# MeteoSwiss/topo-descriptors

Measured on AMD Instinct MI355X. Metric: Mpixels/s (and % HBM roofline) per descriptor, 1/2/4/8 MI355X, higher is better.
Workload: dtype f32

## Files before the change

### topo_descriptors_amd/csrc/disc_ring_wide_impl.hpp

```cpp
#pragma once

namespace topo {

namespace {

constexpr int NCW = 6;

template <int SIZE>
struct WGeo {
    static constexpr DiscTable<SIZE> T = make_disc_table<SIZE>();
    static_assert(T.centre == 0 && T.off_min == -T.off_max, "odd disc sizes only");
    static constexpr int M = T.off_max;
    static constexpr int DL = (M + NCW - 1) / NCW;
    static constexpr int NVL = 64 - 2 * DL;
    static constexpr int TILE_W = NCW * NVL;
    static constexpr int X0 = NCW * DL;
    static constexpr int W = 64 * NCW;
    static constexpr int NR = T.num_runs;
    static_assert(NVL >= 16, "disc too wide for one wavefront");
    struct Sched {
        int first_step[SIZE];
        int order[SIZE];
        int centre_run;
    };
    static constexpr Sched make() {
        Sched t{};
        for (int r = 0; r < SIZE; ++r) t.first_step[r] = -1;
        for (int r = 0; r < SIZE; ++r) t.order[r] = 0;
        t.centre_run = -1;
        for (int D = 0; D <= DL; ++D)
            for (int s = 0; s < NCW; ++s)
                for (int q = 0; q < NCW; ++q) {
                    const int dr = NCW * D + s - q, dl = -NCW * D + s - q;
                    if (dr >= 0 && dr <= M) {
                        const int r = T.run_of[dr - T.off_min];
                        if (D > t.first_step[r]) t.first_step[r] = D;
                    }
                    if (dl < 0 && dl >= -M) {
                        const int r = T.run_of[dl - T.off_min];
                        if (D > t.first_step[r]) t.first_step[r] = D;
                    }
                }
        int n = 0;
        for (int D = DL; D >= 0; --D)
            for (int d = M; d >= 0; --d) {
                const int r = T.run_of[d - T.off_min];
                bool seen = false;
                for (int i = 0; i < n; ++i) seen = seen || t.order[i] == r;
                if (!seen && t.first_step[r] == D) t.order[n++] = r;
            }
        for (int r = 0; r < NR; ++r)
            if (T.run_lo[r] == 0 && T.run_hi[r] == 0) t.centre_run = r;
        return t;
    }
    static constexpr Sched S = make();
    static_assert(S.centre_run >= 0, "the disc's outermost column is the pixel's own row");
};

template <int SIZE>
struct WideCfg {
    using G = WGeo<SIZE>;
    static constexpr int SW = 3;
    static constexpr int CW = 8;
    static constexpr int NW = SW + CW;
    static constexpr int RPW = 2;
    static constexpr int B = CW * RPW;
    static constexpr int TH = 64;
    static constexpr int PPT = TH / B;
    static constexpr int R = SIZE + 2 * B;
    static constexpr int GR = 6;
    static constexpr int HALO = SIZE - 1;
    static constexpr int PAD = 1 + (B - (1 + HALO + B) % B) % B;
    static constexpr int PRO = PAD + HALO + B;
    static constexpr int NB_PRO = PRO / B;
    static constexpr size_t LDS = (size_t)(R + GR) * G::W * sizeof(uint32_t) + 2 * SW * sizeof(int) + 16;
    static_assert(SW * 128 == G::W, "two staged columns per staging lane");
    static_assert(TH % B == 0 && PRO % B == 0, "whole batches");
    static_assert(LDS <= 160 * 1024, "ring does not fit LDS");
    static_assert(NB_PRO <= 15, "batch history: two fields of a flag word");
};

constexpr bool tpi_wide_ring_fits(int size) {
    return size >= 5 && size % 2 == 1 && (size_t)(size + 32 + 6) * 384 * 4 + 64 <= 160 * 1024 && 64 - 2 * ((size / 2 + 5) / 6) >= 16;
}

template <int SIZE, int GR>
struct WBase {
    using G = WGeo<SIZE>;
    static constexpr int NR = G::NR;
    struct Tab {
        int nb;
        int kb[2 * SIZE];
        int first[2 * SIZE];
        int top_b[SIZE], bot_b[SIZE];
        int top_k[SIZE], bot_k[SIZE];
    };
    static constexpr Tab make() {
        Tab t{};
        bool need[2 * SIZE + 2] = {};
        for (int i = 0; i < NR; ++i) {
            const int r = G::S.order[i];
            t.top_k[i] = G::T.run_hi[r] + 1 + G::M;
            t.bot_k[i] = G::T.run_lo[r] + G::M;
            need[t.top_k[i]] = need[t.bot_k[i]] = true;
        }
        t.nb = 0;
        for (int k = 0; k <= 2 * G::M + 1; ++k)
            if (need[k] && (t.nb == 0 || k > t.kb[t.nb - 1] + GR)) t.kb[t.nb++] = k;
        for (int b = 0; b < t.nb; ++b) t.first[b] = NR;
        auto base_of = [&](int k) {
            int b = 0;
            while (b + 1 < t.nb && t.kb[b + 1] <= k) ++b;
            return b;
        };
        for (int i = 0; i < NR; ++i) {
            t.top_b[i] = base_of(t.top_k[i]);
            t.bot_b[i] = base_of(t.bot_k[i]);
            if (i < t.first[t.top_b[i]]) t.first[t.top_b[i]] = i;
            if (i < t.first[t.bot_b[i]]) t.first[t.bot_b[i]] = i;
        }
        return t;
    }
    static constexpr Tab T = make();
    static constexpr bool check() {
        for (int i = 0; i < NR; ++i)
            if (T.top_k[i] - T.kb[T.top_b[i]] > GR || T.top_k[i] < T.kb[T.top_b[i]] || T.bot_k[i] - T.kb[T.bot_b[i]] > GR ||
                T.bot_k[i] < T.kb[T.bot_b[i]])
                return false;
        return true;
    }
    static_assert(check(), "every read within GR rows of its base");
};

#ifndef WIDE_LEAD
#define WIDE_LEAD 2
#endif
#ifndef WIDE_PRIO
#define WIDE_PRIO 1
#endif

typedef uint32_t u32x2w __attribute__((ext_vector_type(2)));
typedef __attribute__((address_space(3))) const char lds_char;
typedef __attribute__((address_space(3))) const volatile u32x2w lds_u32x2w;

template <int SIZE, int R, int GR, int LEAD, bool FIRST>
__device__ __forceinline__ void wide_disc_sum(const uint32_t* ring, int s0, int lane, uint32_t (&acc)[NCW], uint32_t (&ctr)[NCW]) {
    using G = WGeo<SIZE>;
    using BT = WBase<SIZE, GR>;
    constexpr int NR = G::NR;
    constexpr int DL = G::DL;
    constexpr int M = G::M;
    constexpr uint32_t PB = (uint32_t)G::W * 4;
    constexpr uint32_t RB = (uint32_t)R * PB;
    u32x2w top[NR][3], bot[NR][3];
    uint32_t cv[NR][NCW];
    uint32_t aR[NCW], aL[NCW];
    uint32_t vb[BT::T.nb];
    lds_char* q = (lds_char*)ring;
    const uint32_t b0 = (uint32_t)s0 * PB, lb = (uint32_t)lane * (NCW * 4);
    auto fetch = [&](int i) {
        const int r = G::S.order[i];
#pragma unroll
        for (int b = 0; b < BT::T.nb; ++b)
            if (BT::T.first[b] == i) {
                const uint32_t d = b0 + (uint32_t)BT::T.kb[b] * PB;
                vb[b] = lb + min(d, d - RB);
                asm("" : "+v"(vb[b]));
            }
        lds_char* pt = q + vb[BT::T.top_b[i]] + (uint32_t)(BT::T.top_k[i] - BT::T.kb[BT::T.top_b[i]]) * PB;
        lds_char* pb = q + vb[BT::T.bot_b[i]] + (uint32_t)(BT::T.bot_k[i] - BT::T.kb[BT::T.bot_b[i]]) * PB;
#pragma unroll
        for (int h = 0; h < 3; ++h) top[r][h] = *(lds_u32x2w*)(pt + 8 * h);
#pragma unroll
        for (int h = 0; h < 3; ++h) bot[r][h] = *(lds_u32x2w*)(pb + 8 * h);
    };
#pragma unroll
    for (int i = 0; i < LEAD && i < NR; ++i) fetch(i);
#if WIDE_PRIO
    if (FIRST) CHAIN_SETPRIO(3);
    else CHAIN_SETPRIO(1);
#endif
    static_assert(DL >= 1, "the last step (D = 0) closes both chains");
#pragma unroll
    for (int D = DL; D >= 0; --D) {
#if WIDE_PRIO
        if (D == DL / 2) {
            if (FIRST) CHAIN_SETPRIO(2);
            else CHAIN_SETPRIO(0);
        }
#endif
#pragma unroll
        for (int j = 0; j < NR; ++j) {
            if (G::S.first_step[G::S.order[j]] == D) {
                const int r = G::S.order[j];
                if (j + LEAD < NR) fetch(j + LEAD);
                RING_SB();
#pragma unroll
                for (int s = 0; s < NCW; ++s) cv[r][s] = top[r][s / 2][s % 2] - bot[r][s / 2][s % 2];
                RING_SB();
            }
        }
#pragma unroll
        for (int t = 0; t < NCW; ++t) {
            uint32_t pr = 0, pl = 0;
            bool anyr = false, anyl = false;
#pragma unroll
            for (int s = 0; s < NCW; ++s) {
                const int dr = NCW * D + s - t;
                const int dl = -NCW * D + s - t;
                if (dr >= 0 && dr <= M) {
                    const uint32_t c = cv[G::T.run_of[dr - G::T.off_min]][s];
                    pr = anyr ? pr + c : c;
                    anyr = true;
                }
                if (dl < 0 && dl >= -M) {
                    const uint32_t c = cv[G::T.run_of[dl - G::T.off_min]][s];
                    pl = anyl ? pl + c : c;
                    anyl = true;
                }
            }
            if (D == DL) {
                aR[t] = pr;
                aL[t] = pl;
            } else if (D == 0) {
                uint32_t own = anyr && anyl ? pr + pl : anyr ? pr : pl;
                asm("" : "+v"(own));
                own = hop_up(aL[t]) + own;
                asm("" : "+v"(own));
                aR[t] = hop(aR[t]) + own;
                asm("" : "+v"(aR[t]));
            } else {
                if (anyr) {
                    asm("" : "+v"(pr));
                    aR[t] = hop(aR[t]) + pr;
                } else {
                    aR[t] = hop(aR[t]);
                }
                if (anyl) {
                    asm("" : "+v"(pl));
                    aL[t] = hop_up(aL[t]) + pl;
                } else {
                    aL[t] = hop_up(aL[t]);
                }
            }
        }
        RING_SB();
    }
#pragma unroll
    for (int t = 0; t < NCW; ++t) {
        acc[t] = aR[t];
        ctr[t] = cv[G::S.centre_run][t];
    }
}


template <int SIZE>
__global__ __launch_bounds__(WideCfg<SIZE>::NW * 64) void tpi_ring_wide_kernel(WaveArgs p, int tiles_x, int tiles_y, PartRun deal) {
    using G = WGeo<SIZE>;
    using C = WideCfg<SIZE>;
    constexpr int B = C::B, R = C::R, PPT = C::PPT, SW = C::SW, NB_PRO = C::NB_PRO, DL = G::DL;
    constexpr unsigned kWindow = (1u << NB_PRO) - 1u;
    constexpr int kBad = 1, kFracOnly = 1 << 15;
    constexpr unsigned kHistMask = kWindow | kWindow * kFracOnly;
    extern __shared__ __attribute__((aligned(16))) uint32_t lds_u[];
    uint32_t* Q = lds_u;
    int* wflags = reinterpret_cast<int*>(Q + (R + C::GR) * G::W);

    const int nb = (int)gridDim.x;
    const int vb = (nb & 7) ? (int)blockIdx.x : (int)(blockIdx.x & 7) * (nb >> 3) + (int)(blockIdx.x >> 3);
    const int lane = threadIdx.x & 63;
    const int wave = __builtin_amdgcn_readfirstlane((int)(threadIdx.x >> 6));
    const int ntiles = tiles_x * tiles_y;
    const int first = deal.first(vb);
    const int last = min(first + deal.count(vb), ntiles);
    const double inv_nm1 = 1.0 / ((double)G::T.taps - 1.0);
    const int rmin = max(0, p.in_row0), rmax = min(p.gny, p.in_row0 + p.in_rows);
    const bool stager = wave < SW;
    const int scol = 128 * wave + 2 * lane;
    int seen_tiles = 0, seen_frac = 0;

#pragma unroll 1
    for (int pos = first; pos < last;) {
        const int tile0 = pos;
        const int ty0 = tile0 % tiles_y;
        const int run_tiles = min(last - tile0, tiles_y - ty0);
        const int strip = tile0 / tiles_y;
        const int nphase = run_tiles * PPT;
        const int ox0 = strip * G::TILE_W;
        const int oyS = (p.out_row0 / C::TH + ty0) * C::TH;
        const int gx0 = ox0 - G::X0;
        const int gy0 = oyS - G::M - C::PAD;
        const int gcol = gx0 + scol;
        const bool col_ok = stager && gcol >= 0 && gcol < p.nx;
        const float* src = p.in + (col_ok ? gcol : 0);
        auto load_batch = [&](int n0, float2 (&v)[B]) {
#pragma unroll
            for (int r = 0; r < B; ++r) {
                int gy = gy0 + n0 + r;
                gy = min(max(gy, rmin), rmax - 1);
                v[r] = *reinterpret_cast<const float2*>(src + (size_t)(gy - p.in_row0) * p.nx);
            }
        };
        uint32_t run0 = 0, run1 = 0;
        int wslot = 0;
        const uint32_t kLimBits = __float_as_uint(kAbsLim + 1.0f);
        auto stage_batch = [&](int n0, const float2 (&v)[B]) {
            uint32_t amax = 0;
            bool frac = false;
#pragma unroll
            for (int r = 0; r < B; ++r) {
                const int gy = gy0 + n0 + r;
                const bool ok = col_ok && gy >= rmin && gy < rmax;
                const float x0 = ok ? v[r].x : 0.0f, x1 = ok ? v[r].y : 0.0f;
                const int i0 = (int)x0, i1 = (int)x1;
                const uint32_t a0 = __float_as_uint(x0) & 0x7fffffffu, a1 = __float_as_uint(x1) & 0x7fffffffu;
                frac |= x0 != (float)i0 || x1 != (float)i1;
                amax = max(amax, max(a0, a1));
                run0 += (uint32_t)i0;
                run1 += (uint32_t)i1;
                int sl = wslot + r;
                sl = sl >= R ? sl - R : sl;
                const u32x2w v2 = {run0, run1};
                *reinterpret_cast<u32x2w*>(Q + sl * G::W + scol) = v2;
                if (sl < C::GR) *reinterpret_cast<u32x2w*>(Q + (sl + R) * G::W + scol) = v2;
            }
            const bool wild = __builtin_amdgcn_ballot_w64(amax >= kLimBits) != 0;
            const bool any_frac = __builtin_amdgcn_ballot_w64(frac) != 0;
            const bool bad = wild || any_frac;
            const bool fr = !wild && any_frac;
            return (bad ? kBad : 0) | (fr ? kFracOnly : 0);
        };
        auto advance_wslot = [&]() {
            wslot += B;
            wslot = wslot >= R ? wslot - R : wslot;
        };
        unsigned hist = 0;
        auto fold = [&](int parity) {
            int all = 0;
#pragma unroll
            for (int w = 0; w < SW; ++w) all |= wflags[parity * SW + w];
            all = __builtin_amdgcn_readfirstlane(all);
            hist = ((hist << 1) | (unsigned)all) & kHistMask;
        };

        float2 va[B];
        __syncthreads();
        if (stager) {
            int bits = 0;
#pragma unroll 1
            for (int k = 0; k < NB_PRO; ++k) {
                load_batch(k * B, va);
                bits |= stage_batch(k * B, va) << (NB_PRO - 1 - k);
                advance_wslot();
            }
            if (lane == 0) wflags[wave] = bits;
            load_batch(C::PRO, va);
        } else {
            for (int k = 0; k < NB_PRO; ++k) advance_wslot();
        }
        __syncthreads();
        {
            int all = 0;
#pragma unroll
            for (int w = 0; w < SW; ++w) all |= wflags[w];
            hist = (unsigned)__builtin_amdgcn_readfirstlane(all) & kHistMask;
        }

        const int ocol = gx0 + lane * NCW;
        const bool lane_ok = lane >= DL && lane < DL + G::NVL && ocol < p.nx;
        bool tile_frac = false;
#pragma unroll 1
        for (int ph = 0; ph < nphase; ++ph) {
            const bool compute = (hist & kWindow) == 0;
            const int oyA = oyS + ph * B;
            tile_frac = tile_frac || (hist & (kWindow * kFracOnly)) != 0;
            if (!compute) {
                const int r0 = max(oyA, p.out_row0), r1 = min(oyA + B, p.out_row0 + p.out_rows) - 1;
                if (r0 <= r1 && threadIdx.x == 0) {
                    const int base = p.out_row0 / p.map_th;
                    const int mx0 = ox0 / p.map_tw, mx1 = (min(ox0 + G::TILE_W, p.nx) - 1) / p.map_tw;
                    for (int mx = mx0; mx <= mx1; ++mx)
                        for (int my = r0 / p.map_th; my <= r1 / p.map_th; ++my) p.defer[mx * p.map_tiles_y + (my - base)] = kNeedsFraction;
                }
            }
            if (ph % PPT == PPT - 1) {
                ++seen_tiles;
                seen_frac += tile_frac ? 1 : 0;
                tile_frac = false;
            }
            if (stager) {
                const int seen = stage_batch(C::PRO + ph * B, va);
                if (lane == 0) wflags[((ph + 1) & 1) * SW + wave] = seen;
                load_batch(C::PRO + (ph + 1) * B, va);
            } else if (compute) {
                static_assert(C::RPW == 2, "two rows per chain wave: the first and the second priority pair");
#pragma unroll
                for (int k = 0; k < C::RPW; ++k) {
                    const int j = (wave - SW) * C::RPW + k;
                    const int oy = oyA + j;
                    if (oy < p.out_row0 || oy >= p.out_row0 + p.out_rows) continue;
                    const int s0 = (C::PAD - 1 + ph * B + j) % R;
                    uint32_t acc[NCW], ctr[NCW];
                    if (k == 0) wide_disc_sum<SIZE, R, C::GR, WIDE_LEAD, true>(Q, s0, lane, acc, ctr);
                    else wide_disc_sum<SIZE, R, C::GR, WIDE_LEAD, false>(Q, s0, lane, acc, ctr);
                    if (lane_ok) {
                        float* o = p.tpi + (size_t)(oy - p.out_row0) * p.nx + ocol;
                        float out_t[NCW];
#pragma unroll
                        for (int t = 0; t < NCW; ++t) {
                            const int xi = (int)ctr[t];
                            out_t[t] = (float)((double)xi - (double)((int)acc[t] - xi) * inv_nm1);
                        }
#pragma unroll
                        for (int P = 0; P < NCW / 2; ++P)
                            if (ocol + 2 * P < p.nx) *reinterpret_cast<float2*>(o + 2 * P) = make_float2(out_t[2 * P], out_t[2 * P + 1]);
                    }
                }
            }
            advance_wslot();
            __syncthreads();
            fold((ph + 1) & 1);
        }
        pos += run_tiles;
    }
    if (p.report != nullptr && vb == nb / 2 && threadIdx.x == 0) {
        __hip_atomic_store(p.report + 1, (uint32_t)seen_frac, __ATOMIC_RELAXED, __HIP_MEMORY_SCOPE_SYSTEM);
        __hip_atomic_store(p.report, (uint32_t)seen_tiles, __ATOMIC_RELAXED, __HIP_MEMORY_SCOPE_SYSTEM);
    }
}

template <int SIZE>
int launch_ring_wide(const Block& b, float* tpi_out, int map_th, int map_tw) {
    using G = WGeo<SIZE>;
    using C = WideCfg<SIZE>;
    Context& c = ctx();
    TOPO_REQUIRE(c.seams.n == 0, "the wide ring takes single-block calls only");
    WaveArgs a{b.in, tpi_out, nullptr, b.in_rows, b.in_row0, b.gny, b.nx, b.out_row0, b.out_rows,
               nullptr, nullptr, nullptr, 0, 0, 0};
    static int blocks_per_cu = 0;
    if (blocks_per_cu == 0) {
        TOPO_HIP(hipFuncSetAttribute((const void*)tpi_ring_wide_kernel<SIZE>, hipFuncAttributeMaxDynamicSharedMemorySize, (int)C::LDS));
        int nblk = 0;
        TOPO_HIP(hipOccupancyMaxActiveBlocksPerMultiprocessor(&nblk, (const void*)tpi_ring_wide_kernel<SIZE>, C::NW * 64, C::LDS));
        blocks_per_cu = nblk < 1 ? 1 : nblk;
    }
    a.report = dem_memo_report(b);
    WaveParts ps;
    int tiles_x = 0;
    long ntiles = 0;
    TOPO_TRY(make_parts(b, a, C::TH, G::TILE_W, true, false, &ps, &tiles_x, &ntiles, map_th, map_tw));
    TOPO_REQUIRE(ps.n == 1 && ps.a[0].map_th == map_th && ps.a[0].map_tw == map_tw, "wide ring: tile map of another geometry");
    const size_t map_bytes = (size_t)((b.nx + map_tw - 1) / map_tw) * ps.a[0].map_tiles_y;
    TOPO_HIP(hipMemsetAsync(ps.a[0].defer, kTileDone, map_bytes, c.compute));
    const long grid = march_grid(c, blocks_per_cu, ntiles);
    deal_parts(&ps, tiles_x, grid, blocks_per_cu);
    hipLaunchKernelGGL(tpi_ring_wide_kernel<SIZE>, dim3((unsigned)grid), dim3(C::NW * 64), C::LDS, c.compute, ps.a[0], tiles_x, ps.tiles_y[0], ps.run[0]);
    TOPO_HIP(hipGetLastError());
    return TOPO_AMD_OK;
}

}

}
```

Before: 306,200.

## Sum two adjacent output rows per chain wave in one sweep sharing prefix rows

Replaces the per-row disc sum with a paired version that computes two consecutive output rows together. The prefix-sum rows the two rows share are loaded from LDS once, which cuts LDS traffic (55 distinct rows instead of 84 for the 67 px disc). Partial sums are accumulated per run as each run arrives, and the stager and compute paths are split at compile time. It also turns wave priority switching off by default. The cost is more live registers (row buffers plus per-step partials for two rows), which risks spills or lower occupancy.

New measurement: 315,200 (median of 6 runs). 1.03x the previous value.

```diff
diff --git a/topo_descriptors_amd/csrc/disc_ring_wide_impl.hpp b/topo_descriptors_amd/csrc/disc_ring_wide_impl.hpp
--- a/topo_descriptors_amd/csrc/disc_ring_wide_impl.hpp
+++ b/topo_descriptors_amd/csrc/disc_ring_wide_impl.hpp
@@ -85,172 +85,225 @@
 }
 
 template <int SIZE, int GR>
-struct WBase {
+struct WPair {
     using G = WGeo<SIZE>;
     static constexpr int NR = G::NR;
+    static constexpr int NK = 2 * G::M + 3;
     struct Tab {
+        int rows;
         int nb;
-        int kb[2 * SIZE];
-        int first[2 * SIZE];
-        int top_b[SIZE], bot_b[SIZE];
-        int top_k[SIZE], bot_k[SIZE];
+        int kb[NK];
+        int first[NK];
+        int base[NK];
+        int use[SIZE][2][2];
+        int nload[SIZE];
+        int load[SIZE][4];
     };
     static constexpr Tab make() {
         Tab t{};
-        bool need[2 * SIZE + 2] = {};
+        bool need[NK] = {};
         for (int i = 0; i < NR; ++i) {
             const int r = G::S.order[i];
-            t.top_k[i] = G::T.run_hi[r] + 1 + G::M;
-            t.bot_k[i] = G::T.run_lo[r] + G::M;
-            need[t.top_k[i]] = need[t.bot_k[i]] = true;
-        }
-        t.nb = 0;
-        for (int k = 0; k <= 2 * G::M + 1; ++k)
-            if (need[k] && (t.nb == 0 || k > t.kb[t.nb - 1] + GR)) t.kb[t.nb++] = k;
+            for (int w = 0; w < 2; ++w) {
+                t.use[i][w][0] = G::T.run_hi[r] + 1 + G::M + w;
+                t.use[i][w][1] = G::T.run_lo[r] + G::M + w;
+            }
+            for (int w = 0; w < 2; ++w)
+                for (int e = 0; e < 2; ++e) {
+                    const int k = t.use[i][w][e];
+                    if (!need[k]) t.load[i][t.nload[i]++] = k;
+                    need[k] = true;
+                }
+        }
+        for (int k = 0; k < NK; ++k) {
+            if (!need[k]) continue;
+            ++t.rows;
+            if (t.nb == 0 || k > t.kb[t.nb - 1] + GR) t.kb[t.nb++] = k;
+            t.base[k] = t.nb - 1;
+        }
         for (int b = 0; b < t.nb; ++b) t.first[b] = NR;
-        auto base_of = [&](int k) {
-            int b = 0;
-            while (b + 1 < t.nb && t.kb[b + 1] <= k) ++b;
-            return b;
-        };
-        for (int i = 0; i < NR; ++i) {
-            t.top_b[i] = base_of(t.top_k[i]);
-            t.bot_b[i] = base_of(t.bot_k[i]);
-            if (i < t.first[t.top_b[i]]) t.first[t.top_b[i]] = i;
-            if (i < t.first[t.bot_b[i]]) t.first[t.bot_b[i]] = i;
-        }
+        for (int i = NR - 1; i >= 0; --i)
+            for (int n = 0; n < t.nload[i]; ++n) t.first[t.base[t.load[i][n]]] = i;
         return t;
     }
     static constexpr Tab T = make();
     static constexpr bool check() {
-        for (int i = 0; i < NR; ++i)
-            if (T.top_k[i] - T.kb[T.top_b[i]] > GR || T.top_k[i] < T.kb[T.top_b[i]] || T.bot_k[i] - T.kb[T.bot_b[i]] > GR ||
-                T.bot_k[i] < T.kb[T.bot_b[i]])
-                return false;
+        bool loaded[NK] = {};
+        for (int i = 0; i < NR; ++i) {
+            for (int n = 0; n < T.nload[i]; ++n) {
+                const int k = T.load[i][n], b = T.base[k];
+                if (k < T.kb[b] || k - T.kb[b] > GR || T.first[b] > i || loaded[k]) return false;
+                loaded[k] = true;
+            }
+            for (int w = 0; w < 2; ++w)
+                for (int e = 0; e < 2; ++e)
+                    if (!loaded[T.use[i][w][e]]) return false;
+        }
         return true;
     }
-    static_assert(check(), "every read within GR rows of its base");
+    static constexpr int kUnshared = 4 * NR;
+    static_assert(check(), "every row loaded once, before its uses, within GR rows of a base formed by then");
+    static_assert(T.rows < kUnshared, "the pair shares no prefix row");
+    static_assert(SIZE != 67 || T.rows == 55, "67 px: 55 distinct prefix rows a pair (84 unshared)");
+};
+
+template <int N, int I = 0, class F>
+__device__ __forceinline__ void wide_static_for(F&& f) {
+    if constexpr (I < N) {
+        f(std::integral_constant<int, I>{});
+        wide_static_for<N, I + 1>(f);
+    }
+}
+
+template <int SIZE>
+struct WSweep {
+    using G = WGeo<SIZE>;
+    struct Tab {
+        int firstR[G::DL + 1][NCW], firstL[G::DL + 1][NCW];
+    };
+    static constexpr Tab make() {
+        Tab t{};
+        for (int D = 0; D <= G::DL; ++D)
+            for (int o = 0; o < NCW; ++o) t.firstR[D][o] = t.firstL[D][o] = -1;
+        for (int j = G::NR - 1; j >= 0; --j)
+            for (int s = NCW - 1; s >= 0; --s)
+                for (int D = 0; D <= G::DL; ++D)
+                    for (int o = 0; o < NCW; ++o) {
+                        const int dr = NCW * D + s - o, dl = -NCW * D + s - o;
+                        if (dr >= 0 && dr <= G::M && G::T.run_of[dr - G::T.off_min] == G::S.order[j]) t.firstR[D][o] = j * NCW + s;
+                        if (dl < 0 && dl >= -G::M && G::T.run_of[dl - G::T.off_min] == G::S.order[j]) t.firstL[D][o] = j * NCW + s;
+                    }
+        return t;
+    }
+    static constexpr Tab T = make();
+    static constexpr int prio_of(int D) { return 3 - (G::DL - D) * 4 / (G::DL + 1); }
 };
 
 #ifndef WIDE_LEAD
 #define WIDE_LEAD 2
 #endif
 #ifndef WIDE_PRIO
-#define WIDE_PRIO 1
+#define WIDE_PRIO 0
 #endif
 
 typedef uint32_t u32x2w __attribute__((ext_vector_type(2)));
 typedef __attribute__((address_space(3))) const char lds_char;
 typedef __attribute__((address_space(3))) const volatile u32x2w lds_u32x2w;
 
-template <int SIZE, int R, int GR, int LEAD, bool FIRST>
-__device__ __forceinline__ void wide_disc_sum(const uint32_t* ring, int s0, int lane, uint32_t (&acc)[NCW], uint32_t (&ctr)[NCW]) {
+template <int SIZE, int R, int GR, int LEAD, bool PRIO>
+__device__ __forceinline__ void wide_pair_sum(const uint32_t* ring, int s0, int lane, uint32_t (&acc)[2][NCW], uint32_t (&ctr)[2][NCW]) {
     using G = WGeo<SIZE>;
-    using BT = WBase<SIZE, GR>;
+    using PT = WPair<SIZE, GR>;
+    using SW_ = WSweep<SIZE>;
     constexpr int NR = G::NR;
     constexpr int DL = G::DL;
     constexpr int M = G::M;
     constexpr uint32_t PB = (uint32_t)G::W * 4;
     constexpr uint32_t RB = (uint32_t)R * PB;
-    u32x2w top[NR][3], bot[NR][3];
-    uint32_t cv[NR][NCW];
-    uint32_t aR[NCW], aL[NCW];
-    uint32_t vb[BT::T.nb];
+    u32x2w row[PT::NK][3];
+    uint32_t pR[2][DL + 1][NCW], pL[2][DL + 1][NCW];
+    uint32_t aR[2][NCW], aL[2][NCW];
+    uint32_t vb[PT::T.nb];
     lds_char* q = (lds_char*)ring;
     const uint32_t b0 = (uint32_t)s0 * PB, lb = (uint32_t)lane * (NCW * 4);
-    auto fetch = [&](int i) {
-        const int r = G::S.order[i];
-#pragma unroll
-        for (int b = 0; b < BT::T.nb; ++b)
-            if (BT::T.first[b] == i) {
-                const uint32_t d = b0 + (uint32_t)BT::T.kb[b] * PB;
+    auto fetch = [&](auto I) {
+        constexpr int i = decltype(I)::value;
+#pragma unroll
+        for (int b = 0; b < PT::T.nb; ++b)
+            if (PT::T.first[b] == i) {
+                const uint32_t d = b0 + (uint32_t)PT::T.kb[b] * PB;
                 vb[b] = lb + min(d, d - RB);
                 asm("" : "+v"(vb[b]));
             }
-        lds_char* pt = q + vb[BT::T.top_b[i]] + (uint32_t)(BT::T.top_k[i] - BT::T.kb[BT::T.top_b[i]]) * PB;
-        lds_char* pb = q + vb[BT::T.bot_b[i]] + (uint32_t)(BT::T.bot_k[i] - BT::T.kb[BT::T.bot_b[i]]) * PB;
-#pragma unroll
-        for (int h = 0; h < 3; ++h) top[r][h] = *(lds_u32x2w*)(pt + 8 * h);
-#pragma unroll
-        for (int h = 0; h < 3; ++h) bot[r][h] = *(lds_u32x2w*)(pb + 8 * h);
+#pragma unroll
+        for (int n = 0; n < PT::T.nload[i]; ++n) {
+            const int k = PT::T.load[i][n];
+            lds_char* pk = q + vb[PT::T.base[k]] + (uint32_t)(k - PT::T.kb[PT::T.base[k]]) * PB;
+#pragma unroll
+            for (int h = 0; h < 3; ++h) row[k][h] = *(lds_u32x2w*)(pk + 8 * h);
+        }
     };
-#pragma unroll
-    for (int i = 0; i < LEAD && i < NR; ++i) fetch(i);
-#if WIDE_PRIO
-    if (FIRST) CHAIN_SETPRIO(3);
-    else CHAIN_SETPRIO(1);
-#endif
-    static_assert(DL >= 1, "the last step (D = 0) closes both chains");
-#pragma unroll
-    for (int D = DL; D >= 0; --D) {
-#if WIDE_PRIO
-        if (D == DL / 2) {
-            if (FIRST) CHAIN_SETPRIO(2);
-            else CHAIN_SETPRIO(0);
-        }
-#endif
-#pragma unroll
-        for (int j = 0; j < NR; ++j) {
-            if (G::S.first_step[G::S.order[j]] == D) {
-                const int r = G::S.order[j];
-                if (j + LEAD < NR) fetch(j + LEAD);
-                RING_SB();
-#pragma unroll
-                for (int s = 0; s < NCW; ++s) cv[r][s] = top[r][s / 2][s % 2] - bot[r][s / 2][s % 2];
-                RING_SB();
-            }
-        }
-#pragma unroll
-        for (int t = 0; t < NCW; ++t) {
+    auto close = [&](auto DD) {
+        constexpr int D = decltype(DD)::value;
+        wide_static_for<NCW * 2>([&](auto TW) {
+            constexpr int t = decltype(TW)::value / 2, w = decltype(TW)::value % 2;
+            constexpr bool anyr = SW_::T.firstR[D][t] >= 0, anyl = SW_::T.firstL[D][t] >= 0;
             uint32_t pr = 0, pl = 0;
-            bool anyr = false, anyl = false;
-#pragma unroll
-            for (int s = 0; s < NCW; ++s) {
-                const int dr = NCW * D + s - t;
-                const int dl = -NCW * D + s - t;
-                if (dr >= 0 && dr <= M) {
-                    const uint32_t c = cv[G::T.run_of[dr - G::T.off_min]][s];
-                    pr = anyr ? pr + c : c;
-                    anyr = true;
-                }
-                if (dl < 0 && dl >= -M) {
-                    const uint32_t c = cv[G::T.run_of[dl - G::T.off_min]][s];
-                    pl = anyl ? pl + c : c;
-                    anyl = true;
-                }
-            }
-            if (D == DL) {
-                aR[t] = pr;
-                aL[t] = pl;
-            } else if (D == 0) {
+            if constexpr (anyr) pr = pR[w][D][t];
+            if constexpr (anyl) pl = pL[w][D][t];
+            if constexpr (D == DL) {
+                aR[w][t] = pr;
+                aL[w][t] = pl;
+            } else if constexpr (D == 0) {
                 uint32_t own = anyr && anyl ? pr + pl : anyr ? pr : pl;
                 asm("" : "+v"(own));
-                own = hop_up(aL[t]) + own;
+                own = hop_up(aL[w][t]) + own;
                 asm("" : "+v"(own));
-                aR[t] = hop(aR[t]) + own;
-                asm("" : "+v"(aR[t]));
+                aR[w][t] = hop(aR[w][t]) + own;
+                asm("" : "+v"(aR[w][t]));
             } else {
-                if (anyr) {
+                if constexpr (anyr) {
                     asm("" : "+v"(pr));
-                    aR[t] = hop(aR[t]) + pr;
+                    aR[w][t] = hop(aR[w][t]) + pr;
                 } else {
-                    aR[t] = hop(aR[t]);
-                }
-                if (anyl) {
+                    aR[w][t] = hop(aR[w][t]);
+                }
+                if constexpr (anyl) {
                     asm("" : "+v"(pl));
-                    aL[t] = hop_up(aL[t]) + pl;
+                    aL[w][t] = hop_up(aL[w][t]) + pl;
                 } else {
-                    aL[t] = hop_up(aL[t]);
-                }
-            }
-        }
+                    aL[w][t] = hop_up(aL[w][t]);
+                }
+            }
+        });
         RING_SB();
-    }
-#pragma unroll
-    for (int t = 0; t < NCW; ++t) {
-        acc[t] = aR[t];
-        ctr[t] = cv[G::S.centre_run][t];
-    }
+    };
+    wide_static_for<(LEAD < NR ? LEAD : NR)>([&](auto I) { fetch(I); });
+    if constexpr (PRIO) CHAIN_SETPRIO(3);
+    static_assert(DL >= 1 && G::S.first_step[G::S.order[0]] == DL, "the first run opens the chains, the last step (D = 0) closes both");
+    wide_static_for<NR>([&](auto J) {
+        constexpr int j = decltype(J)::value;
+        constexpr int r = G::S.order[j];
+        constexpr int D = G::S.first_step[r];
+        constexpr int Dprev = j == 0 ? DL : G::S.first_step[G::S.order[j > 0 ? j - 1 : 0]];
+        constexpr int Dnext = j + 1 < NR ? G::S.first_step[G::S.order[j + 1 < NR ? j + 1 : j]] : -1;
+        if constexpr (PRIO && SW_::prio_of(D) != SW_::prio_of(Dprev)) CHAIN_SETPRIO(SW_::prio_of(D));
+        if constexpr (j + LEAD < NR) fetch(std::integral_constant<int, j + LEAD>{});
+        RING_SB();
+        wide_static_for<NCW>([&](auto S) {
+            constexpr int s = decltype(S)::value;
+            uint32_t cv[2];
+#pragma unroll
+            for (int w = 0; w < 2; ++w) {
+                cv[w] = row[PT::T.use[j][w][0]][s / 2][s % 2] - row[PT::T.use[j][w][1]][s / 2][s % 2];
+                if (r == G::S.centre_run) ctr[w][s] = cv[w];
+            }
+            wide_static_for<(DL + 1) * NCW>([&](auto ET) {
+                constexpr int E = decltype(ET)::value / NCW, t = decltype(ET)::value % NCW;
+                constexpr int dr = NCW * E + s - t, dl = -NCW * E + s - t;
+                if constexpr (dr >= 0 && dr <= M) {
+                    if constexpr (G::T.run_of[dr - G::T.off_min] == r) {
+                        static_assert(E <= D, "a run arrives at the first step that takes it");
+#pragma unroll
+                        for (int w = 0; w < 2; ++w) pR[w][E][t] = SW_::T.firstR[E][t] == j * NCW + s ? cv[w] : pR[w][E][t] + cv[w];
+                    }
+                }
+                if constexpr (dl < 0 && dl >= -M) {
+                    if constexpr (G::T.run_of[dl - G::T.off_min] == r) {
+                        static_assert(E <= D, "a run arrives at the first step that takes it");
+#pragma unroll
+                        for (int w = 0; w < 2; ++w) pL[w][E][t] = SW_::T.firstL[E][t] == j * NCW + s ? cv[w] : pL[w][E][t] + cv[w];
+                    }
+                }
+            });
+        });
+        RING_SB();
+        wide_static_for<D - Dnext>([&](auto C) { close(std::integral_constant<int, D - decltype(C)::value>{}); });
+    });
+#pragma unroll
+    for (int w = 0; w < 2; ++w)
+#pragma unroll
+        for (int t = 0; t < NCW; ++t) acc[w][t] = aR[w][t];
 }
 
 
@@ -343,9 +396,13 @@
             hist = ((hist << 1) | (unsigned)all) & kHistMask;
         };
 
-        float2 va[B];
+        const int ocol = gx0 + lane * NCW;
+        const bool lane_ok = lane >= DL && lane < DL + G::NVL && ocol < p.nx;
         __syncthreads();
-        if (stager) {
+        auto run_phases = [&](auto STG) {
+        constexpr bool stg = decltype(STG)::value;
+        float2 va[stg ? B : 1];
+        if constexpr (stg) {
             int bits = 0;
 #pragma unroll 1
             for (int k = 0; k < NB_PRO; ++k) {
@@ -366,8 +423,6 @@
             hist = (unsigned)__builtin_amdgcn_readfirstlane(all) & kHistMask;
         }
 
-        const int ocol = gx0 + lane * NCW;
-        const bool lane_ok = lane >= DL && lane < DL + G::NVL && ocol < p.nx;
         bool tile_frac = false;
 #pragma unroll 1
         for (int ph = 0; ph < nphase; ++ph) {
@@ -388,32 +443,33 @@
                 seen_frac += tile_frac ? 1 : 0;
                 tile_frac = false;
             }
-            if (stager) {
+            if constexpr (stg) {
                 const int seen = stage_batch(C::PRO + ph * B, va);
                 if (lane == 0) wflags[((ph + 1) & 1) * SW + wave] = seen;
                 load_batch(C::PRO + (ph + 1) * B, va);
             } else if (compute) {
-                static_assert(C::RPW == 2, "two rows per chain wave: the first and the second priority pair");
-#pragma unroll
-                for (int k = 0; k < C::RPW; ++k) {
-                    const int j = (wave - SW) * C::RPW + k;
-                    const int oy = oyA + j;
-                    if (oy < p.out_row0 || oy >= p.out_row0 + p.out_rows) continue;
+                static_assert(C::RPW == 2, "a chain wave sums its two rows of a phase in one sweep");
+                const int j = (wave - SW) * C::RPW;
+                const int oy = oyA + j;
+                if (oy + C::RPW > p.out_row0 && oy < p.out_row0 + p.out_rows) {
                     const int s0 = (C::PAD - 1 + ph * B + j) % R;
-                    uint32_t acc[NCW], ctr[NCW];
-                    if (k == 0) wide_disc_sum<SIZE, R, C::GR, WIDE_LEAD, true>(Q, s0, lane, acc, ctr);
-                    else wide_disc_sum<SIZE, R, C::GR, WIDE_LEAD, false>(Q, s0, lane, acc, ctr);
-                    if (lane_ok) {
-                        float* o = p.tpi + (size_t)(oy - p.out_row0) * p.nx + ocol;
-                        float out_t[NCW];
-#pragma unroll
-                        for (int t = 0; t < NCW; ++t) {
-                            const int xi = (int)ctr[t];
-                            out_t[t] = (float)((double)xi - (double)((int)acc[t] - xi) * inv_nm1);
+                    uint32_t acc[C::RPW][NCW], ctr[C::RPW][NCW];
+                    wide_pair_sum<SIZE, R, C::GR, WIDE_LEAD, WIDE_PRIO != 0>(Q, s0, lane, acc, ctr);
+#pragma unroll
+                    for (int k = 0; k < C::RPW; ++k) {
+                        const bool row_ok = oy + k >= p.out_row0 && oy + k < p.out_row0 + p.out_rows;
+                        if (lane_ok && row_ok) {
+                            float* o = p.tpi + (size_t)(oy + k - p.out_row0) * p.nx + ocol;
+                            float out_t[NCW];
+#pragma unroll
+                            for (int t = 0; t < NCW; ++t) {
+                                const int xi = (int)ctr[k][t];
+                                out_t[t] = (float)((double)xi - (double)((int)acc[k][t] - xi) * inv_nm1);
+                            }
+#pragma unroll
+                            for (int P = 0; P < NCW / 2; ++P)
+                                if (ocol + 2 * P < p.nx) *reinterpret_cast<float2*>(o + 2 * P) = make_float2(out_t[2 * P], out_t[2 * P + 1]);
                         }
-#pragma unroll
-                        for (int P = 0; P < NCW / 2; ++P)
-                            if (ocol + 2 * P < p.nx) *reinterpret_cast<float2*>(o + 2 * P) = make_float2(out_t[2 * P], out_t[2 * P + 1]);
                     }
                 }
             }
@@ -421,6 +477,9 @@
             __syncthreads();
             fold((ph + 1) & 1);
         }
+        };
+        if (stager) run_phases(std::true_type{});
+        else run_phases(std::false_type{});
         pos += run_tiles;
     }
     if (p.report != nullptr && vb == nb / 2 && threadIdx.x == 0) {
```
